# qwang-sj/qwen3-asr.cpp

Measured on AMD Instinct MI355X. Metric: RTFx (audio-sec/wall-sec) + decode tokens/sec, Qwen3-ASR-0.6B f16, higher is better.
Workload: dtype f16

## Files before the change

### qwen3-asr.cpp_amd/csrc/attention.hip

```cpp
#include <algorithm>
#include <type_traits>
#include <cstdlib>
#include <stdexcept>

#include "dev_common.h"
#include "fx_chain.h"
#include "fx_decode.h"
#include "kernels.h"

namespace qasr {

#define EKS 66
#define EVS 68

__global__ __launch_bounds__(256) void enc_attn_kernel(const float *__restrict__ qkv, const int *__restrict__ seg_start,
                                                       const int *__restrict__ seg_len, int D, uint16_t *__restrict__ out,
                                                       float *__restrict__ out32) {
    __shared__ __attribute__((aligned(16))) float Ks[64 * EKS];
    __shared__ __attribute__((aligned(16))) float Vs[64 * EVS];
    const int b = blockIdx.z, h = blockIdx.y;
    const int N = seg_len[b], r0 = seg_start[b];
    const int qblk = blockIdx.x * 64;
    if (qblk >= N) return;
    const int tid = threadIdx.x, lane = tid & 63, wid = tid >> 6;
// ... 512 lines not shown
#pragma unroll
                for (int i = 0; i < 4; i++) dst[d * 16 + 4 * g + i] = f_to_u16(o[d][i] * inv);
        }
    }
}

void launch_prefill_attention(const PrefillAttnArgs &a, hipStream_t s) {
    if (a.n_seq <= 0 || a.max_len <= 0) return;
    dim3 grid((a.max_len + 31) / 32, a.n_kv_head, a.n_seq);
    hipLaunchKernelGGL(prefill_attn_kernel, grid, dim3(256), 0, s, a);
}

#define DSPLIT 64
#define DWAVES 4

__device__ __forceinline__ void st_sc1_x4(float *p, float4 f) {
    const floatx4 v = {f.x, f.y, f.z, f.w};
    asm volatile("global_store_dwordx4 %0, %1, off sc1" ::"v"(p), "v"(v) : "memory");
}
__device__ __forceinline__ void ld_sc1_x4_burst5(const floatx4 *src, int tid, int n4, floatx4 *v) {
    const floatx4 *p[5];
#pragma unroll
    for (int j = 0; j < 5; j++) p[j] = src + min(tid + 256 * j, n4 - 1);
    asm volatile(
        "global_load_dwordx4 %0, %5, off sc1\n\t"
        "global_load_dwordx4 %1, %6, off sc1\n\t"
        "global_load_dwordx4 %2, %7, off sc1\n\t"
        "global_load_dwordx4 %3, %8, off sc1\n\t"
        "global_load_dwordx4 %4, %9, off sc1\n\t"
        "s_waitcnt vmcnt(0)"
        : "=&v"(v[0]), "=&v"(v[1]), "=&v"(v[2]), "=&v"(v[3]), "=&v"(v[4])
        : "v"(p[0]), "v"(p[1]), "v"(p[2]), "v"(p[3]), "v"(p[4])
        : "memory");
}
__device__ __forceinline__ void ld_sc1_x4_4(const uint16_t *p, u32x4 *v) {
    asm volatile(
        "global_load_dwordx4 %0, %4, off sc1\n\t"
        "global_load_dwordx4 %1, %4, off offset:1024 sc1\n\t"
        "global_load_dwordx4 %2, %4, off offset:2048 sc1\n\t"
        "global_load_dwordx4 %3, %4, off offset:3072 sc1\n\t"
        "s_waitcnt vmcnt(0)"
        : "=&v"(v[0]), "=&v"(v[1]), "=&v"(v[2]), "=&v"(v[3])
        : "v"(p)
        : "memory");
}

__device__ __forceinline__ half8 kv_load(const uint16_t *p, int nt) {
    return nt ? __builtin_nontemporal_load((const half8 *)p) : *(const half8 *)p;
}

template <int SPL>
struct alignas(16) SplitLds {
    uint16_t qs[2][128];
    uint16_t knew[128];
    uint16_t vnew[128];
    float sc[2][SPL];
    float ored[DWAVES * 4][2][128];
    float cml[2][2];
    int last;
};
template <int SPL, bool FUSED>
__device__ __forceinline__ void decode_attn_body(const DecodeAttnArgs a, const int sp, const int g, const int b, const int nsp,
                                                 SplitLds<SPL> &SL) {
    auto &qs = SL.qs;
    auto &knew = SL.knew;
    auto &vnew = SL.vnew;
    auto &sc = SL.sc;
    auto &ored = SL.ored;
    auto &cml = SL.cml;
    auto &last = SL.last;
    const int tid = threadIdx.x, lane = tid & 63, wid = tid >> 6;
    const int QD = a.n_head * 128, KD = a.n_kv_head * 128;
    const long blk = sp + (long)nsp * (g + (long)a.n_kv_head * b);
    auto mark = [&](int slot) {
        if (a.trace && tid == 0) a.trace[blk * 8 + slot] = rt_now();
    };
    mark(0);
    const float *raw = a.qkv + (long)b * (QD + 2 * KD);
    const float *src = wid < 2 ? raw + (2 * g + wid) * 128 : raw + QD + (wid - 2) * KD + g * 128;
    float x0 = 0.f, x1 = 0.f;
    if constexpr (!FUSED) { x0 = src[lane]; x1 = src[lane + 64]; }
    const float *nw = wid < 2 ? a.q_norm : a.k_norm;
    const float w0 = nw[lane], w1 = nw[lane + 64];
    if constexpr (FUSED)
        for (int i = 0; i < a.fuse_delay; i++) __builtin_amdgcn_s_sleep(8);
    const long cbase = ((long)b * a.n_kv_head + g) * a.max_ctx;
    uint16_t *kc = a.kc + cbase * 128, *vc = a.vc + cbase * 128;
    const int k0 = sp * SPL;
    const int sub = lane >> 4, dl = (lane & 15) * 8;
    const int q4 = lane >> 4, c16 = lane & 15;
    constexpr int KPW = SPL / DWAVES / 4;
    constexpr int TW = SPL / DWAVES / 16;
    const int kcap = FUSED ? a.max_ctx - 1 : min(a.pos[b], a.max_ctx - 1);
    half8 kk[TW][4], vv[KPW];
#pragma unroll
    for (int t = 0; t < TW; t++)
#pragma unroll
        for (int s4 = 0; s4 < 4; s4++) {
            const int key = min(k0 + wid * (SPL / DWAVES) + 16 * t + c16, kcap);
            kk[t][s4] = kv_load(kc + (long)key * 128 + 32 * s4 + 8 * q4, a.kv_nt);
        }
    if (FUSED && a.fx) {
        if (a.fx_vpf & 1) {
            const uint16_t *vt = a.vt + ((long)b * a.n_kv_head + g) * 128 * vt_ctx(a.max_ctx) + (long)(k0 / 8) * 1024;
#pragma unroll
            for (int i = 0; i < KPW; i++) vv[i] = *(const half8 *)(vt + (long)(i * 256 + tid) * 8);
        }
    } else if (!a.scores) {
#pragma unroll
        for (int i = 0; i < KPW; i++) {
            const int key = min(k0 + wid * (SPL / DWAVES) + i * 4 + sub, kcap);
            vv[i] = kv_load(vc + (long)key * 128 + dl, a.kv_nt);
        }
    }
    if (FUSED && a.gran) {
        const uint32_t tag = gran_tag(a.pos[b], a.layer);
        const unsigned long long *gp = a.gran + (src - raw) + lane;
        unsigned long long v0 = 0, v1 = 0;
        bool ok = false;
        for (int it = 0; it < a.poll_limit; it++) {
            v0 = __hip_atomic_load(gp, __ATOMIC_RELAXED, __HIP_MEMORY_SCOPE_AGENT);
            v1 = __hip_atomic_load(gp + 64, __ATOMIC_RELAXED, __HIP_MEMORY_SCOPE_AGENT);
            ok = (uint32_t)(v0 >> 32) == tag && (uint32_t)(v1 >> 32) == tag;
            if (__all(ok)) break;
            __builtin_amdgcn_s_sleep(2);
        }
        if (!__all(ok) && lane == 0) __hip_atomic_fetch_or(a.err, (unsigned)DEVERR_QKV_WAIT, __ATOMIC_RELAXED, __HIP_MEMORY_SCOPE_AGENT);
        x0 = __uint_as_float((uint32_t)v0);
        x1 = __uint_as_float((uint32_t)v1);
    } else if constexpr (FUSED) {
        if (tid == 0) {
            int ok = 0;
            for (int it = 0; it < a.poll_limit; it++) {
                if (__hip_atomic_load(a.qcnt + (g * 8 + (sp & 7)) * 16, __ATOMIC_RELAXED, __HIP_MEMORY_SCOPE_AGENT) >=
                    (a.qkv_need ? a.qkv_need : 64u)) {
                    ok = 1;
                    break;
                }
                __builtin_amdgcn_s_sleep(4);
            }
            if (a.fence) {
                __builtin_amdgcn_fence(__ATOMIC_ACQUIRE, "agent");
                asm volatile("s_waitcnt vmcnt(0)" ::: "memory");
            }
            if (!ok) __hip_atomic_fetch_or(a.err, (unsigned)DEVERR_QKV_WAIT, __ATOMIC_RELAXED, __HIP_MEMORY_SCOPE_AGENT);
        }
        __syncthreads();
        const uint32_t *sr = (const uint32_t *)src;
        x0 = __uint_as_float(__hip_atomic_load(sr + lane, __ATOMIC_RELAXED, __HIP_MEMORY_SCOPE_AGENT));
        x1 = __uint_as_float(__hip_atomic_load(sr + lane + 64, __ATOMIC_RELAXED, __HIP_MEMORY_SCOPE_AGENT));
    }
    const int pos = a.pos[b];
    const int nkv = pos + 1;
    const int k1 = min(nkv, k0 + SPL);
    const bool lastsp = sp == (nkv - 1) / SPL;
    const float2 cs = *(const float2 *)(a.rope + ((long)pos * 64 + lane) * 2);
    if (wid < 3) {
        const double ss = wave_sum_d((double)(x0 * x0) + (double)(x1 * x1));
        const float scale = 1.0f / sqrtf((float)(ss / 128.0) + a.eps);
        const float y0 = fmul_rn(fmul_rn(x0, scale), w0), y1 = fmul_rn(fmul_rn(x1, scale), w1);
        const uint16_t r0 = f_to_u16(y0 * cs.x - y1 * cs.y), r1 = f_to_u16(y0 * cs.y + y1 * cs.x);
        if (wid < 2) {
            qs[wid][lane] = r0;
            qs[wid][lane + 64] = r1;
        } else if (lastsp) {
            knew[lane] = r0; knew[lane + 64] = r1;
            kc[(long)pos * 128 + lane] = r0;
            kc[(long)pos * 128 + lane + 64] = r1;
        }
    } else if (lastsp) {
        const uint16_t v0 = f_to_u16(x0), v1 = f_to_u16(x1);
        vnew[lane] = v0; vnew[lane + 64] = v1;
        vc[(long)pos * 128 + lane] = v0;
        vc[(long)pos * 128 + lane + 64] = v1;
        uint16_t *t = a.vt + ((long)b * a.n_kv_head + g) * 128 * vt_ctx(a.max_ctx);
        t[vt_index(pos, lane)] = v0;
        t[vt_index(pos, lane + 64)] = v1;
    }
    __syncthreads();
    if (a.trace) { asm volatile("s_waitcnt vmcnt(0)" ::: "memory"); mark(1); }
    half8 qa[4];
#pragma unroll
    for (int s4 = 0; s4 < 4; s4++)
        qa[s4] = c16 < 2 ? *(const half8 *)&qs[c16][32 * s4 + 8 * q4] : half8{0, 0, 0, 0, 0, 0, 0, 0};
#pragma unroll
    for (int t = 0; t < TW; t++) {
        const int j = wid * (SPL / DWAVES) + 16 * t + c16;
        if (k0 + j == pos)
#pragma unroll
            for (int s4 = 0; s4 < 4; s4++) kk[t][s4] = *(const half8 *)&knew[32 * s4 + 8 * q4];
        floatx4 acc = {0.f, 0.f, 0.f, 0.f};
#pragma unroll
        for (int s4 = 0; s4 < 4; s4++) acc = __builtin_amdgcn_mfma_f32_16x16x32_f16(qa[s4], kk[t][s4], acc, 0, 0, 0);
        if (q4 == 0) {
            const bool ok = k0 + j < k1;
            sc[0][j] = ok ? acc[0] * a.scale : -INFINITY;
            sc[1][j] = ok ? acc[1] * a.scale : -INFINITY;
        }
    }
#pragma unroll
    for (int i = 0; i < KPW; i++) {
        const int j = wid * (SPL / DWAVES) + i * 4 + sub;
        if (k0 + j == pos) vv[i] = *(const half8 *)&vnew[dl];
    }
    __syncthreads();
    mark(6);
    if constexpr (FUSED) {
        if (a.fx) {
            const uint32_t tag = gran_tag(pos, a.layer);
            if (tid < 2 * SPL) {
                const int hh = tid / SPL, j = tid - hh * SPL;
                if (k0 + j < k1)
// ... 457 lines not shown
        fx_weights2(p ? fmaxf(Mp0, lh) : Mp0, p ? sv[2] : sv[0], p ? sv[3] : sv[1], x0, x1);
        const int k = k0 + 2 * p;
        if (k == kl) { C.fwl = x0; x0 = 0.0f; }
        if (k + 1 == kl) { C.fwl = x1; x1 = 0.0f; }
        *(float2 *)&C.fsc[(k >> 5) * FX_ST + (k & 31)] = make_float2(x0, x1);
        uint32_t m16 = kb << (4 * (lane & 3));
        m16 |= __shfl_xor(m16, 1, 64);
        m16 |= __shfl_xor(m16, 2, 64);
        const uint32_t bits = fx_chunk_bits(kb);
        if (p == 0) {
            if ((lane & 3) == 0) C.kmask[ch * (FX_PC / 16) + (lane >> 2)] = (uint16_t)m16;
            if ((lane & 7) == 7) C.gmax[ch * (FX_PC / DX_B) + (lane >> 3)] = Mi;
        }
        __builtin_amdgcn_fence(__ATOMIC_RELEASE, "workgroup");
        if (lane == 0) __hip_atomic_store(pb + 4 * ch + p, (unsigned char)(0x80u | bits), __ATOMIC_RELAXED, __HIP_MEMORY_SCOPE_WORKGROUP);
        if (tr && p == 0 && lane == 0 && (ch == 0 || ch == nch - 1)) {
            if (ch == 0) tr[2] = rt_now();
            if (ch == nch - 1) tr[3] = rt_now();
        }
    }
    if (p != 0) return;
    {
        uint32_t w = 0;
        for (int it = 0; it < a.poll_limit; it++) {
            w = __hip_atomic_load(pb + 4 * (nch - 1) + 1, __ATOMIC_RELAXED, __HIP_MEMORY_SCOPE_WORKGROUP);
            if (w & 0x80u) break;
            __builtin_amdgcn_s_sleep(1);
        }
        if (!(w & 0x80u) && lane == 0) __hip_atomic_fetch_or(a.err, (unsigned)DEVERR_SCORE_WAIT, __ATOMIC_RELAXED, __HIP_MEMORY_SCOPE_AGENT);
        __builtin_amdgcn_fence(__ATOMIC_ACQUIRE, "workgroup");
    }
    float term = 0.0f;
    if (lane * DX_B < nch * FX_PC) {
        const float *row = C.fsc + lane * FX_ST;
        const float wl = C.fwl;
        float Sl = 0.0f;
#pragma unroll
        for (int i = 0; i < DX_B; i += 4) {
            const floatx4 r = *(const floatx4 *)&row[i];
#pragma unroll
            for (int e = 0; e < 4; e++) Sl = __builtin_signbit(r[e]) ? fadd_rn(fmul_rn(Sl, -r[e]), 1.0f) : fadd_rn(fmul_rn(Sl, 1.0f), r[e]);
        }
        if (lane == (kl >> 5)) Sl = __builtin_signbit(wl) ? fadd_rn(fmul_rn(Sl, -wl), 1.0f) : fadd_rn(fmul_rn(Sl, 1.0f), wl);
        const float Ml = C.gmax[lane];
        term = Ml == -INFINITY ? 0.0f : Sl * expf(Ml - M);
    }
    const float S = wave_sum(term);
    if (lane == 0) C.S = S;
    __builtin_amdgcn_fence(__ATOMIC_RELEASE, "workgroup");
    if (lane == 0) __hip_atomic_store(&C.prog[DX_KC / FX_PC], FX_PUB, __ATOMIC_RELAXED, __HIP_MEMORY_SCOPE_WORKGROUP);
    if (tr && lane == 0) {
        tr[6] = rt_now();
        tr[7] = npoll;
    }
}
__device__ __forceinline__ uint32_t fx1_progress(const DecodeAttnArgs &a, ChainLds &C, const int i) {
    const uint32_t *pw = &C.prog[i];
    uint32_t w = (uint32_t)__builtin_amdgcn_readfirstlane((int)__hip_atomic_load(pw, __ATOMIC_RELAXED, __HIP_MEMORY_SCOPE_WORKGROUP));
    if (__builtin_expect((w & FX_PUB) != FX_PUB, 0)) {
        for (int it = 0; it < a.poll_limit; it++) {
            __builtin_amdgcn_s_sleep(1);
            w = (uint32_t)__builtin_amdgcn_readfirstlane((int)__hip_atomic_load(pw, __ATOMIC_RELAXED, __HIP_MEMORY_SCOPE_WORKGROUP));
            if ((w & FX_PUB) == FX_PUB) break;
        }
        if ((w & FX_PUB) != FX_PUB && (threadIdx.x & 63) == 0)
            __hip_atomic_fetch_or(a.err, (unsigned)DEVERR_SCORE_WAIT, __ATOMIC_RELAXED, __HIP_MEMORY_SCOPE_AGENT);
    }
    __builtin_amdgcn_fence(__ATOMIC_ACQUIRE, "workgroup");
    return w;
}
__device__ __forceinline__ void fx1_chain_body(const DecodeAttnArgs &a, const int c, ChainLds &C) {
    const int tid = threadIdx.x, lane = tid & 63, wid = __builtin_amdgcn_readfirstlane(tid >> 6);
    const int g = c % a.n_kv_head, hh = c / a.n_kv_head, head = 2 * g + hh;
    const int wu = wid & 1;
    const int d = 64 * wu + lane, loff = 8 * lane;
    const uint16_t *vt = a.vt + (long)g * 128 * vt_ctx(a.max_ctx) + 64 * wu * 8;
    unsigned long long *tr = a.trace ? a.trace + (4000L + c) * 8 : nullptr;
    auto mark = [&](int slot) {
        if (tr && tid == 0) tr[slot] = rt_now();
    };
    mark(0);
    const int pos = a.pos[0], n = pos + 1;
    if (tid <= DX_KC / FX_PC) C.prog[tid] = 0u;
    if (a.fx_vpf & 2) {
        typedef __attribute__((address_space(3))) void lds_void_c;
        typedef __attribute__((address_space(1))) void glb_void_c;
        lds_void_c *dst = (lds_void_c *)C.vpf[wid];
        for (int kb = wid >> 1; kb * 8 < n; kb += 2)
            __builtin_amdgcn_global_load_lds((glb_void_c *)(vt + (long)kb * 1024 + loff), dst, 16, 0, 0);
    }
    __syncthreads();
    if (wid >= 2) {
        fx1_gather_weights(a, head, n, C, wid - 2, tr);
    } else {
        const uint32_t tag = gran_tag(pos, a.layer);
        const int QD = a.n_head * 128, KD = a.n_kv_head * 128;
        const float *fsc = C.fsc;
        const uint16_t *kmask = C.kmask;
        const int nl = n - 1;
        if (a.trace && nl > 0) {
            (void)fx1_progress(a, C, 0);
            mark(1);
        }
        const unsigned long long ck0 = a.trace ? clock64() : 0ull;
        f16 acc = 0;
        {
            u32x4 va[DX_Q / 8], vb[DX_Q / 8];
            floatx4 wa, wb;
            const int lastb = nl > 0 ? (nl - 1) >> 3 : 0;
            const int nfull = nl > 0 ? (lastb + 1) >> 3 : 0;
            constexpr uint32_t QB = DX_Q / 8 * 2048;
            const __amdgpu_buffer_rsrc_t vrs = __builtin_amdgcn_make_buffer_rsrc((void *)vt, (short)0, lastb * 2048 + 1024, 0x00020000);
            const uint32_t voff = 16 * lane;
            int jt = 0;
            fx_loadQ(va, vt, loff, 0, lastb);
            uint32_t bm = 0;
            const float *wrow = fsc;
            const uint16_t *krow = kmask;
            for (; jt + 2 * DX_Q < nfull * DX_Q; jt += 2 * DX_Q, bm >>= 2, wrow += 2 * DX_Q / DX_B * FX_ST, krow += 2 * DX_Q / 16) {
                fx_loadQ_sb(vb, vrs, voff, (jt / DX_Q + 1) * QB);
                if ((jt & (FX_PC - 1)) == 0) {
                    bm = fx1_progress(a, C, jt / FX_PC);
                    fx_w8(wrow, 0, wa, wb);
                }
                fx_step1_lds_b(va, 0, wrow, krow, bm & 1u, acc, wa, wb);
                fx_loadQ_sb(va, vrs, voff, (jt / DX_Q + 2) * QB);
                fx_step1_lds_b(vb, DX_Q, wrow, krow, bm & 2u, acc, wa, wb);
            }
            for (int j0 = jt; j0 < nl; j0 += 2 * DX_Q, bm >>= 2) {
                fx_loadQ(vb, vt, loff, j0 + DX_Q, lastb);
                if ((j0 & (FX_PC - 1)) == 0) {
                    bm = fx1_progress(a, C, j0 / FX_PC);
                    fx_w8(fsc, j0, wa, wb);
                }
                fx_step1_lds_b(va, j0, fsc, kmask, bm & 1u, acc, wa, wb);
                if (j0 + DX_Q >= nl) break;
                fx_loadQ(va, vt, loff, j0 + 2 * DX_Q, lastb);
                fx_step1_lds_b(vb, j0 + DX_Q, fsc, kmask, bm & 2u, acc, wa, wb);
            }
        }
        const unsigned long long ck1 = a.trace ? clock64() : 0ull;
        uint16_t vnew = 0;
        {
            const unsigned long long *gp = a.gran + QD + KD + g * 128 + d;
            unsigned long long v = 0;
            bool ok = false;
            for (int it = 0; it < a.poll_limit; it++) {
                v = __hip_atomic_load(gp, __ATOMIC_RELAXED, __HIP_MEMORY_SCOPE_AGENT);
                ok = (uint32_t)(v >> 32) == tag;
                if (__all(ok)) break;
                __builtin_amdgcn_s_sleep(2);
            }
            if (!__all(ok) && lane == 0) __hip_atomic_fetch_or(a.err, (unsigned)DEVERR_QKV_WAIT, __ATOMIC_RELAXED, __HIP_MEMORY_SCOPE_AGENT);
            vnew = f_to_u16(__uint_as_float((uint32_t)v));
        }
        (void)fx1_progress(a, C, DX_KC / FX_PC);
        const float S = C.S;
        acc = fx_key_slow(acc, vnew, C.fwl);
        mark(4);
        if (a.trace && lane == 0) {
            a.trace[(4080L + c) * 8 + wid] = rt_now();
            a.trace[(4080L + c) * 8 + 2 + wid] = ck1 - ck0;
        }
        if (a.trace && tid == 0) {
            a.trace[(4040L + c) * 8 + 0] = ck0;
            a.trace[(4040L + c) * 8 + 1] = ck1;
            a.trace[(4040L + c) * 8 + 2] = (unsigned long long)n;
        }
        const float ov = (float)acc * (S == 0.0f ? 0.0f : 1.0f / S);
        const uint32_t h16 = f_to_u16(ov);
        const uint32_t hn = __shfl_xor(h16, 1, 64);
        uint16_t *out = a.out + head * 128 + d;
        if (a.att_done) {
            if ((lane & 1) == 0) __hip_atomic_store((uint32_t *)out, h16 | (hn << 16), __ATOMIC_RELAXED, __HIP_MEMORY_SCOPE_AGENT);
            asm volatile("s_waitcnt vmcnt(0)" ::: "memory");
        } else {
            *out = (uint16_t)h16;
        }
    }
    if (a.att_done) {
        __syncthreads();
        if (a.fence && tid == 0) {
            __builtin_amdgcn_fence(__ATOMIC_RELEASE, "agent");
            asm volatile("s_waitcnt vmcnt(0)" ::: "memory");
        }
        if (a.fence) __syncthreads();
        if (tid < 8) __hip_atomic_fetch_add(a.att_done + tid * 16, 1u, __ATOMIC_RELAXED, __HIP_MEMORY_SCOPE_AGENT);
    }
    mark(5);
    if (a.trace && tid == 0) {
        unsigned nk = 0, ng = 0;
        for (int i = 0; i < (n + FX_PC - 1) / FX_PC * (FX_PC / 16); i++) {
            const unsigned m = C.kmask[i];
            nk += __builtin_popcount(m);
            ng += ((m & 0xffu) != 0) + ((m >> 8) != 0);
        }
        a.trace[(4040L + c) * 8 + 3] = nk;
        a.trace[(4040L + c) * 8 + 4] = ng;
    }
}

template <int SPL>
__global__ __launch_bounds__(256) void qkv_attn1_kernel(GemvArgs q, DecodeAttnArgs a, GemvArgs o) {
    constexpr int K = 1024, NT = 2, RPW = 2;
    constexpr size_t RLB = sizeof(SplitLds<SPL>) > sizeof(ChainLds) ? sizeof(SplitLds<SPL>) : sizeof(ChainLds);
    __shared__ __attribute__((aligned(16))) unsigned char role_lds[RLB];
    stamp_start(a.stamp);
    if (blockIdx.x >= 512) {
        const int j = blockIdx.x - 512, nsp = a.grid_splits, nat = nsp * a.n_kv_head;
        const int nfx = fx_chain_wgs(a.fx, a.n_head);
        if (j >= nat + nfx) oproj1_body(o, a, j - nat - nfx);
        else if (j >= nat) fx1_chain_body(a, j - nat, *reinterpret_cast<ChainLds *>(role_lds));
        else decode_attn_body<SPL, true>(a, j / a.n_kv_head, j % a.n_kv_head, 0, nsp, *reinterpret_cast<SplitLds<SPL> *>(role_lds));
        stamp_end(a.stamp);
        return;
    }
    const int lane = threadIdx.x & 63, wid = threadIdx.x >> 6;
    const int grp = blockIdx.x >> 6, loc = blockIdx.x & 63;
    if (q.trace && threadIdx.x == 0) q.trace[blockIdx.x * 8] = rt_now();
    const int QD = a.n_head * 128, KD = a.n_kv_head * 128;
    const int rbase = loc < 32 ? grp * 256 + loc * 8 : loc < 48 ? QD + grp * 128 + (loc - 32) * 8 : QD + KD + grp * 128 + (loc - 48) * 8;
    const int row0 = rbase + wid * RPW;
    const uint32_t gtag = a.gran ? gran_tag(a.pos[0], a.layer) : 0u;
    half8 wv[RPW][NT];
#pragma unroll
    for (int r = 0; r < RPW; r++)
#pragma unroll
        for (int t = 0; t < NT; t++)
            wv[r][t] = __builtin_nontemporal_load((const half8 *)(q.W + (long)(row0 + r) * K + t * 512 + lane * 8));
    float xf[NT][8];
    if (q.embd_ids) {
        const uint16_t *er = q.embd + (long)q.embd_ids[0] * K;
#pragma unroll
        for (int t = 0; t < NT; t++) {
            const half8 h = *(const half8 *)(er + t * 512 + lane * 8);
#pragma unroll
            for (int e = 0; e < 8; e++) xf[t][e] = (float)h[e];
        }
        if (q.x_store && blockIdx.x == 0 && wid == 0)
#pragma unroll
            for (int t = 0; t < NT; t++)
#pragma unroll
                for (int e = 0; e < 8; e++)
                    __hip_atomic_store((uint32_t *)(q.x_store + t * 512 + lane * 8 + e), __float_as_uint(xf[t][e]), __ATOMIC_RELAXED,
                                       __HIP_MEMORY_SCOPE_AGENT);
    } else {
#pragma unroll
        for (int t = 0; t < NT; t++) {
            const float4 u = *(const float4 *)(q.x + t * 512 + lane * 8);
            const float4 v = *(const float4 *)(q.x + t * 512 + lane * 8 + 4);
            xf[t][0] = u.x; xf[t][1] = u.y; xf[t][2] = u.z; xf[t][3] = u.w;
            xf[t][4] = v.x; xf[t][5] = v.y; xf[t][6] = v.z; xf[t][7] = v.w;
        }
    }
    double ss = 0.0;
#pragma unroll
    for (int t = 0; t < NT; t++)
#pragma unroll
        for (int e = 0; e < 8; e++) ss += (double)(xf[t][e] * xf[t][e]);
    ss = wave_sum_d(ss);
    const float scale = 1.0f / sqrtf((float)(ss / K) + q.eps);
#pragma unroll
    for (int t = 0; t < NT; t++) {
        const float4 u = *(const float4 *)(q.norm_w + t * 512 + lane * 8);
        const float4 v = *(const float4 *)(q.norm_w + t * 512 + lane * 8 + 4);
        const float w[8] = {u.x, u.y, u.z, u.w, v.x, v.y, v.z, v.w};
#pragma unroll
        for (int e = 0; e < 8; e++) xf[t][e] = (float)f2h(fmul_rn(fmul_rn(xf[t][e], scale), w[e]));
    }
#pragma unroll
    for (int r = 0; r < RPW; r++) {
        float acc = 0.f;
#pragma unroll
        for (int t = 0; t < NT; t++)
#pragma unroll
            for (int e = 0; e < 8; e++) acc = fmaf((float)wv[r][t][e], xf[t][e], acc);
        acc = wave_sum(acc);
        if (a.gran) {
            if (lane == 0)
                __hip_atomic_store(a.gran + row0 + r, ((unsigned long long)gtag << 32) | __float_as_uint(acc), __ATOMIC_RELAXED,
                                   __HIP_MEMORY_SCOPE_AGENT);
        } else if (lane == 0) {
            __hip_atomic_store((uint32_t *)(q.out_f32 + row0 + r), __float_as_uint(acc), __ATOMIC_RELAXED, __HIP_MEMORY_SCOPE_AGENT);
        }
    }
    if (a.gran) {
        if (q.trace && threadIdx.x == 0) q.trace[blockIdx.x * 8 + 1] = rt_now();
        stamp_end(a.stamp);
        return;
    }
    asm volatile("s_waitcnt vmcnt(0)" ::: "memory");
    __syncthreads();
    if (a.fence && threadIdx.x == 0) {
        __builtin_amdgcn_fence(__ATOMIC_RELEASE, "agent");
        asm volatile("s_waitcnt vmcnt(0)" ::: "memory");
    }
    if (a.fence) __syncthreads();
    if (threadIdx.x < 8)
        __hip_atomic_fetch_add(a.qcnt + (grp * 8 + threadIdx.x) * 16, 1u, __ATOMIC_RELAXED, __HIP_MEMORY_SCOPE_AGENT);
    if (q.trace && threadIdx.x == 0) q.trace[blockIdx.x * 8 + 1] = rt_now();
    stamp_end(a.stamp);
}

static int split1(int spl1, int grid_splits) { return spl1 == 64 || spl1 == 128 ? spl1 : grid_splits >= 30 ? 128 : 64; }

int launch_qkv_attention1(const GemvArgs &q, const DecodeAttnArgs &a, const GemvArgs *o, const FuseCfg &cfg, hipStream_t s, bool dry) {
    if (!cfg.qkv || !cfg.err || a.B != 1 || !a.qcnt || q.M != 1 || q.K != 1024 || q.Wd || !q.norm_w || q.xh || q.bias || q.res ||
        a.out32 || a.outq || q.N != a.n_head * 128 + 2 * a.n_kv_head * 128 || a.n_head != 2 * a.n_kv_head || a.n_kv_head * 64 != 512)
        return 0;
    const int spl1 = split1(cfg.spl1, a.grid_splits);
    const int ns = (a.grid_splits * DSPLIT + spl1 - 1) / spl1;
    const bool with_o = cfg.o && o && a.att_done && o->M == 1 && o->K == 2048 && o->N == 1024 && o->xh && o->res &&
                        !o->Wd && !o->bias && !o->norm_w && o->xh == a.out;
    if (a.fx && (!a.gran || !a.sgran || ns * spl1 > DX_KC)) return 0;
    const int nfx = fx_chain_wgs(a.fx, a.n_head);
    const int slots = spl1 == 128 ? cfg.slots_qkv128 : cfg.slots_qkv64;
    const int o_blocks = 1024 / OPROJ_ROWS;
    const bool fit_o = 512 + ns * a.n_kv_head + nfx + o_blocks <= slots;
    if (512 + ns * a.n_kv_head + nfx > slots) return 0;
    const bool with_o2 = with_o && fit_o;
    if (dry) return with_o2 ? 2 : 1;
    const dim3 grid(512 + ns * a.n_kv_head + nfx + (with_o2 ? o_blocks : 0));
    DecodeAttnArgs ad = a;
    ad.fuse_delay = cfg.qkv_delay;
    ad.oproj_delay = cfg.o_delay;
    ad.poll_limit = cfg.poll_limit;
    ad.fence = cfg.fence;
    ad.err = cfg.err;
    ad.grid_splits = ns;
    ad.fx_vpf = cfg.fx_vpf;
    if (!with_o2) ad.att_done = nullptr;
    const GemvArgs qa = q;
    const GemvArgs oa = with_o2 ? *o : GemvArgs{};
    if (spl1 == 128) hipLaunchKernelGGL(qkv_attn1_kernel<128>, grid, dim3(256), 0, s, qa, ad, oa);
    else hipLaunchKernelGGL(qkv_attn1_kernel<DSPLIT>, grid, dim3(256), 0, s, qa, ad, oa);
    return with_o2 ? 2 : 1;
}

void launch_decode_attention(const DecodeAttnArgs &a, hipStream_t s) {
    if (a.B <= 0) return;
    if (a.B <= 8) {
        if (split1(a.spl1, a.grid_splits) == 128) {
            const int g2 = (a.grid_splits * DSPLIT + 127) / 128;
            hipLaunchKernelGGL(decode_attn_kernel<128>, dim3(g2, a.n_kv_head, a.B), dim3(256), 0, s, a);
        } else {
            hipLaunchKernelGGL(decode_attn_kernel<DSPLIT>, dim3(a.grid_splits, a.n_kv_head, a.B), dim3(256), 0, s, a);
        }
    } else if (a.stream_blocks > 0 && a.n_head == 2 * a.n_kv_head && a.n_kv_head * a.B >= a.stream_blocks / 2) {
        hipLaunchKernelGGL(decode_attn_seq_kernel<0>, dim3(a.n_kv_head, a.B), dim3(256), 0, s, a);
    } else {
        if (a.spl_batch == 128) {
            const int g2 = (a.grid_splits * DSPLIT + 127) / 128;
            hipLaunchKernelGGL(decode_attn_kernel<128>, dim3(g2, a.n_kv_head, a.B), dim3(256), 0, s, a);
        } else {
            const int g4 = (a.grid_splits * DSPLIT + 255) / 256;
            hipLaunchKernelGGL(decode_attn_kernel<256>, dim3(g4, a.n_kv_head, a.B), dim3(256), 0, s, a);
        }
    }
}

bool launch_decode_attention_exact_seq(const DecodeAttnArgs &a, hipStream_t s) {
    const size_t lds = (size_t)2 * a.max_ctx * sizeof(float);
    if (!a.fx_seq || a.B <= 8 || a.stream_blocks <= 0 || a.n_head != 2 * a.n_kv_head || a.n_kv_head * a.B < a.stream_blocks / 2 ||
        lds > 32768)
        return false;
    hipLaunchKernelGGL(decode_attn_seq_kernel<1>, dim3(a.n_kv_head, a.B), dim3(256), lds, s, a);
    return true;
}

int fused_slots_ffn();

void fused_slots(FuseCfg &cfg) {
    auto slots_of = [](const void *kernel) {
        int nb = 0, dev = 0, cus = 0;
        if (hipGetDevice(&dev) != hipSuccess || hipDeviceGetAttribute(&cus, hipDeviceAttributeMultiprocessorCount, dev) != hipSuccess ||
            hipOccupancyMaxActiveBlocksPerMultiprocessor(&nb, kernel, 256, 0) != hipSuccess)
            return 0;
        return nb * cus;
    };
    cfg.slots_qkv64 = slots_of(reinterpret_cast<const void *>(qkv_attn1_kernel<DSPLIT>));
    cfg.slots_qkv128 = slots_of(reinterpret_cast<const void *>(qkv_attn1_kernel<128>));
    cfg.slots_ffn = fused_slots_ffn();
    cfg.slots_stream = decode_stream_slots();
}

int decode_split_len() { return DSPLIT; }
int decode_max_splits() { return 256; }

}
```

### qwen3-asr.cpp_amd/csrc/engine.hip

```cpp
#include <memory>

#include "engine_impl.h"

using namespace qasr;
using namespace qasr::eng;

static thread_local std::string g_err;

int qasr::eng::fail(int code, const std::string &msg) {
    g_err = msg;
    return code;
}

int qasr::eng::declined_check(const char *stage) {
    std::string msg;
    if (qasr::take_declined(&msg)) return fail(QASR_ERR_STATE, std::string(stage) + ": " + msg);
    return 0;
}

struct FuseOption {
    const char *name, *env;
    int FuseCfg::*field;
};
static const std::vector<FuseOption> &fuse_options() {
    static const std::vector<FuseOption> v = {
        {"fuse_ffn", "QASR_FUSE_FFN", &FuseCfg::ffn},          {"fuse_qkv", "QASR_FUSE_QKV", &FuseCfg::qkv},
        {"fuse_o", "QASR_FUSE_O", &FuseCfg::o},
        {"ffn_delay", "QASR_FFN_DELAY", &FuseCfg::ffn_delay},
        {"ffn_wdelay", "QASR_FFN_WDELAY", &FuseCfg::ffn_wdelay}, {"qkv_delay", "QASR_FUSE_DELAY", &FuseCfg::qkv_delay},
        {"o_delay", "QASR_FUSE_ODELAY", &FuseCfg::o_delay},    {"att_spl1", "QASR_ATT_SPL1", &FuseCfg::spl1},
        {"poll_limit", "QASR_POLL_LIMIT", &FuseCfg::poll_limit}, {"handoff_fence", "QASR_HANDOFF_FENCE", &FuseCfg::fence},
        {"fa_exact_prefill", "QASR_FA_EXACT_PREFILL", &FuseCfg::fa_exact_prefill},
        {"enc_attn_f32", "QASR_ENC_ATTN_F32", &FuseCfg::enc_attn_f32},
        {"gemm_regs", "QASR_GEMM_REGS", &FuseCfg::gemm_regs},
        {"gran", "QASR_GRAN", &FuseCfg::gran},
        {"fa_exact_decode", "QASR_FA_EXACT_DECODE", &FuseCfg::fa_exact_decode},
        {"fx_vpf", "QASR_FX_VPF", &FuseCfg::fx_vpf},
        {"att_stream", "QASR_ATT_STREAM", &FuseCfg::att_stream},
        {"skinny", "QASR_SKINNY", &FuseCfg::skinny},
        {"att_spl", "QASR_ATT_SPL", &FuseCfg::att_spl},
        {"kv_nt", "QASR_KV_NT", &FuseCfg::kv_nt},
        {"lmh", "QASR_LMH", &FuseCfg::lmh},
        {"fx_seq", "QASR_FX_SEQ", &FuseCfg::fx_seq},
        {"skinny_inf", "QASR_SKINNY_INF", &FuseCfg::skinny_inf},
        {"skinny_wdef", "QASR_SKINNY_WDEF", &FuseCfg::skinny_wdef},
        {"refill_group", "QASR_REFILL_GROUP", &FuseCfg::refill_group},
        {"live_prefix", "QASR_LIVE_PREFIX", &FuseCfg::live_prefix},
        {"staged_wrap", "QASR_STAGED_WRAP", &FuseCfg::staged_wrap},
        {"poison_scratch", "QASR_POISON_SCRATCH", &FuseCfg::poison},
        {"token_logprobs", "QASR_TOKEN_LOGPROBS", &FuseCfg::token_logprobs},
        {"top_k", "QASR_TOP_K", &FuseCfg::top_k},
        {"lmh_topk", "QASR_LMH_TOPK", &FuseCfg::lmh_topk},
        {"beam_width", "QASR_BEAM_WIDTH", &FuseCfg::beam_width},
        {"sample_slices", "QASR_SAMPLE_SLICES", &FuseCfg::sample_slices},
    };
    return v;
}

int qasr::eng::reset_counters(qasr_ctx *c) {
    HIPCHK(hipMemsetAsync(c->d_ffncnt, 0, c->ffncnt_bytes(), c->st));
    HIPCHK(hipMemsetAsync(c->d_qcnt, 0, c->qcnt_bytes(), c->st));
    HIPCHK(hipMemsetAsync(c->d_attdone, 0, c->attdone_bytes(), c->st));
    HIPCHK(hipMemsetAsync(c->d_counter, 0, c->counter_bytes(), c->st));
    HIPCHK(hipMemsetAsync(c->d_done, 0, qasr_ctx::kDoneBytes, c->st));
    HIPCHK(hipMemsetAsync(c->d_amax, 0, c->amax_bytes(), c->st));
    return 0;
}

int qasr::eng::reset_granules(qasr_ctx *c) {
    HIPCHK(hipMemsetAsync(c->d_gran, 0, c->gran_bytes(), c->st));
    HIPCHK(hipMemsetAsync(c->d_sgran, 0, c->sgran_bytes(), c->st));
    return 0;
}

int qasr::eng::check_dev_err(qasr_ctx *c) {
    unsigned e = 0;
    HIPCHK(hipMemcpyAsync(&e, c->d_err, 4, hipMemcpyDeviceToHost, c->st));
    HIPCHK(hipStreamSynchronize(c->st));
    if (!e) return 0;
    HIPCHK(hipMemsetAsync(c->d_err, 0, 4, c->st));
    const int rc = reset_counters(c);
    if (rc) return rc;
    HIPCHK(hipStreamSynchronize(c->st));
    std::string what;
    if (e & DEVERR_QKV_WAIT) what += " attention<-QKV";
    if (e & DEVERR_O_WAIT) what += " o-proj<-attention";
    if (e & DEVERR_FFN_WAIT) what += " down<-gate/up";
    if (e & DEVERR_SCORE_WAIT) what += " chain<-scores";
    return fail(QASR_ERR_DEVICE, "fused decode launch: an in-launch wait timed out (" + what.substr(1) +
                                     "); outputs of this call are invalid (another process or context sharing the GPU?)");
}

std::mutex &qasr::eng::device_lock(int device) {
    static std::mutex m[64];
    return m[(unsigned)device % 64];
}

int qasr::eng::dev_alloc(qasr_ctx *c, void **p, size_t bytes) {
    HIPCHK(hipMalloc(p, bytes ? bytes : 256));
    c->owned.push_back({*p, bytes});
    return 0;
}

int qasr::eng::ensure(qasr_ctx *c, DevBuf &b, size_t bytes) {
    if (b.n >= bytes && b.p) return 0;
    if (b.p) {
        HIPCHK(hipStreamSynchronize(c->st));
        for (auto it = c->owned.begin(); it != c->owned.end(); ++it)
            if (it->p == b.p) { c->owned.erase(it); break; }
        HIPCHK(hipFree(b.p));
        b.p = nullptr;
    }
    size_t n = std::max<size_t>(bytes + bytes / 4, 4096);
    HIPCHK(hipMalloc(&b.p, n));
    b.n = n;
    c->owned.push_back({b.p, n});
    if (c->fuse.poison) HIPCHK(hipMemsetAsync(b.p, 0xFF, n, c->st));
    return 0;
}

// ... 329 lines not shown
```

### qwen3-asr.cpp_amd/csrc/kernels.h

```cpp
#pragma once

#include <string>

#include <hip/hip_runtime.h>
#include <stdint.h>

namespace qasr {

struct MelClip {
    long pcm_off;
    int n;
    int TF;
    long tmp_off;
    long out_off;
};
void launch_mel(const float *pcm, const MelClip *clips, int n_clips, const int2 *blocks, int n_blocks,
                const double2 *tw, const double *hann, const float *filt, double *tmp, unsigned long long *cmax,
                float *out, hipStream_t s);
int mel_frames_per_block();

struct ResampleClip {
    long in_off;
    long out_off;
    int n_in, n_out;
// ... 38 lines not shown
    const uint16_t *A; int lda;
    const uint16_t *W; int ldw;
    int M, N, K;
    const ChunkDesc *chunks; const int *row_start; int n_chunks; int C;
    const float *bias;
    const float *res; int ldr;
    float *out_f32; int ldo;
    uint16_t *out_f16; int ldo16;
    const uint16_t *gelu;
    const float *pe; const int *pe_pos;
    unsigned long long *amax;
    int n_valid;
    const int8_t *Aq; const float *Ad; int ldad;
    const int8_t *Wq; const uint16_t *Wd;
    int regs_staged;
    int no_skinny;
    int skinny_inflight;
    int8_t *out_q; float *out_d; int ldoq;
    int wdef;
};
void launch_gemm(int amode, int epi, const GemmArgs &g, hipStream_t s);
void note_declined(const char *what, int mode, int epi);
void note_declined_shape(const char *what, int M, int N, int K);
bool take_declined(std::string *msg);
void note_kernel(const char *family, int n, int a = 0, int b = 0, int c = 0, int d = 0, int e = 0);
bool take_kernel(std::string *tag);
bool launch_gemm_skinny(int epi, const GemmArgs &g, hipStream_t s);
bool launch_gemm_skinny_q8(int epi, const GemmArgs &g, hipStream_t s);
void launch_gemm_q8(int epi, const GemmArgs &g, hipStream_t s);
void launch_quantize_q8(const float *x32, const uint16_t *x16, int ldx, int M, int K, int gather_C, int8_t *q, float *d,
                        hipStream_t s);

struct ScoreHeadArgs {
    const uint16_t *A; int lda;
    const uint16_t *W; int ldw;
    int R, N, K, n_valid;
    const int32_t *target;
    float *lp;
    int32_t *gid;
    float *glp;
    void *scratch;
    int cols_fast;
};
size_t score_head_scratch(int R, int N);
bool launch_score_head(const ScoreHeadArgs &a, hipStream_t s);

struct GemvArgs {
    const float *x; int ldx;
    const uint16_t *xh; int ldxh;
    const float *norm_w; float eps;
    const uint16_t *W; int K, N, M;
    const uint16_t *Wd;
    const float *bias;
    const float *res; int ldr;
    float *out_f32; int ldo;
    uint16_t *out_f16; int ldo16;
    unsigned long long *amax;
    const int32_t *embd_ids; const uint16_t *embd; float *x_store;
    unsigned int *done; int32_t *tok_out; int32_t *hist; int hist_stride; int *step; int *pos;
    unsigned long long *trace;
    unsigned int *zero8;
    unsigned long long *stamp;
    int *nkv;
    int n_valid;
    int keep_step;
    unsigned long long *lp_part; float *lp_out; float *lp_hist;
    unsigned long long *tk_part; int32_t *tk_out; float *tk_lp; int32_t *tk_hist; float *tk_lphist; int tk_k;
};
void launch_gemv(int epi, const GemvArgs &g, hipStream_t s);
bool launch_lmhead_batch(const GemvArgs &g, hipStream_t s);
int lmhead_grid();
bool launch_gemv1(int epi, const GemvArgs &g, hipStream_t s);

enum DevErr : unsigned {
    DEVERR_QKV_WAIT = 1u,
    DEVERR_O_WAIT = 2u,
    DEVERR_FFN_WAIT = 4u,
    DEVERR_SCORE_WAIT = 8u,
};
struct FuseCfg {
    int ffn = 1, qkv = 1, o = 1;
    int ffn_delay = 4, ffn_wdelay = 16;
    int qkv_delay = 10, o_delay = 32;
    int spl1 = 0;
    int poll_limit = 1 << 20;
    int fence = 0;
    int enc_attn_f32 = 0;
    int gemm_regs = 0;
    int gran = 1;
    int fa_exact_prefill = 1;
    int fa_exact_decode = 1;
    int fx_vpf = 2;
    int slots_ffn = 0, slots_qkv64 = 0, slots_qkv128 = 0;
    int att_stream = 1;
    int skinny = 1;
    int att_spl = 256;
    int kv_nt = 1;
    int slots_stream = 0;
    int fx_seq = 1;
    int lmh = 1;
    int skinny_inf = 1;
    int skinny_wdef = 1;
    int refill_group = 0;
    int live_prefix = 0;
    int staged_wrap = 0;
    int poison = 0;
    int sample_slices = 0;
    int token_logprobs = 0;
    int lmh_topk = 1;
    int top_k = 0;
    int beam_width = 0;
    unsigned int *err = nullptr;
};
void fused_slots(FuseCfg &cfg);
struct FfnCtl {
    unsigned int *cnt, *cnt_next;
    unsigned int *err;
    int wdelay, delay, poll_limit, fence;
};
bool launch_ffn1(const GemvArgs &gu, const GemvArgs &dn, unsigned int *cnt, unsigned int *cnt_next, const FuseCfg &cfg,
                 hipStream_t s, bool dry = false);

void launch_layernorm_f16(const float *x, int M, int D, const float *w, const float *b, float eps, uint16_t *y, hipStream_t s,
                          float *y32 = nullptr);
void launch_rmsnorm_f16(const float *x, int ldx, const int *row_idx, int M, int D, const float *w, float eps,
                        uint16_t *y, hipStream_t s, float *y32 = nullptr);
void launch_rmsnorm_q8(const float *x, int ldx, int M, int D, const float *w, float eps, int8_t *yq, float *yd, hipStream_t s);

void launch_enc_attention(const float *qkv, const int *seg_start, const int *seg_len, int n_seg, int max_len,
                          int D, int H, uint16_t *out, hipStream_t s, float *out32 = nullptr, bool f32_mfma = false);

constexpr long kKvPadRows = 256;
__host__ __device__ inline int vt_ctx(int max_ctx) { return (max_ctx + 63) / 64 * 64 + 384; }
__host__ __device__ inline long vt_index(int k, int d) { return ((long)(k >> 3) * 128 + d) * 8 + (k & 7); }

struct QkvPostArgs {
    const float *qkv; int rows;
    const int *row_seq; const int *row_pos;
    const float *q_norm, *k_norm; float eps;
    const float *rope;
    int n_head, n_kv_head;
    uint16_t *q_out;
    uint16_t *kc, *vc;
    int max_ctx;
    uint16_t *vt;
    float *q32, *k32;
};
void launch_qkv_post(const QkvPostArgs &a, hipStream_t s);

struct PrefillAttnArgs {
    const uint16_t *q;
    const uint16_t *kc, *vc;
    const int *seq_row0; const int *seq_len; const int *seq_slot; int n_seq; int max_len;
    int n_head, n_kv_head, max_ctx;
    float scale;
    uint16_t *out;
    float *out32;
    int8_t *outq; float *outd;
    const float *q32, *k32;
    const int *seq_pos0;
};
void launch_prefill_attention(const PrefillAttnArgs &a, hipStream_t s);
void launch_prefill_attention_exact(const PrefillAttnArgs &a, hipStream_t s);
hipError_t check_expf_nonpos(unsigned long long *mismatches);

__host__ __device__ inline int sgran_ld(int max_ctx) { return (max_ctx + 63) / 64 * 64; }
__host__ __device__ inline uint32_t gran_tag(int pos, int layer) { return ((uint32_t)(pos + 1) << 5) | (uint32_t)layer; }

struct DecodeAttnArgs {
    const float *qkv;
    const float *q_norm, *k_norm; float eps;
    const float *rope;
    const int *pos;
    uint16_t *kc, *vc;
    uint16_t *vt;
    const int *seq_slot;
    int B, n_head, n_kv_head, max_ctx, max_splits;
    int grid_splits;
    float scale;
    float *part;
    unsigned int *counter;
    uint16_t *out;
    float *out32;
    int8_t *outq; float *outd;
    unsigned long long *trace;
    unsigned int *qcnt;
    int fuse_delay;
    unsigned int *att_done;
    int oproj_delay;
    int poll_limit;
    int fence;
    unsigned int *err;
    int spl1;
    unsigned long long *stamp;
    unsigned int qkv_need;
    float *scores;
    unsigned long long *gran;
    int layer;
    int stream_blocks;
    int spl_batch;
    int kv_nt;
    int fx_seq;
    int fx;
    unsigned long long *sgran;
    int fx_vpf;
};
void launch_decode_attention_exact(const DecodeAttnArgs &a, hipStream_t s);
bool launch_decode_attention_exact_seq(const DecodeAttnArgs &a, hipStream_t s);

void launch_decode_attention(const DecodeAttnArgs &a, hipStream_t s);
int launch_qkv_attention1(const GemvArgs &q, const DecodeAttnArgs &a, const GemvArgs *o, const FuseCfg &cfg, hipStream_t s,
                          bool dry = false);
int decode_split_len();
int decode_max_splits();

void launch_embed(const int32_t *ids, int rows, const uint16_t *embd, int hidden, const float *audio,
                  const int *row_audio , float *x, hipStream_t s);
void launch_argmax_finish(const unsigned long long *amax, int B, int32_t *ids, int32_t *hist, int hist_stride,
                          const int *step, hipStream_t s);
void launch_fill_u64(unsigned long long *p, int n, unsigned long long v, hipStream_t s);
void launch_token_logprob(const float *logits, int ld, int B, int n_valid, const int32_t *tok, const int *step, float *lp_out,
                          float *lp_hist, int hist_stride, hipStream_t s, int src_div = 1);
constexpr int TOPK_MAX = 8;
bool launch_topk_rows(const float *logits, int ld, int B, int n_valid, int K, const int *step, int32_t *tk_ids, float *tk_lp,
                      int32_t *tk_hist_ids, float *tk_hist_lp, int hist_stride, hipStream_t s);
void launch_gather_rows(const float *src, const int *idx, int rows, int D, float *dst, hipStream_t s);
void launch_step_advance(int *row_pos, int *n_kv, int *step, int B, hipStream_t s);

struct KvForkArgs {
    uint16_t *kc, *vc, *vt;
    int layers, n_kv_head, max_ctx, slots;
    const int *parent, *from, *to;
    int B, group, blocks;
};
bool launch_kv_fork(const KvForkArgs &a, hipStream_t s);
struct BeamSelectArgs {
    const int32_t *tk_id; const float *tk_lp;
    float *cum;
    int *fin_row, *fin_t; float *fin_sum, *fin_lp;
    int *n_fin, *done, *t;
    const int *P;
    int32_t *tok;
    int *parent, *from, *to;
    int *h_par; int32_t *h_id; float *h_lp;
    int hist_stride, hist_base;
    int W, G;
    const int32_t *eos;
};
bool launch_beam_select(const BeamSelectArgs &a, hipStream_t s);

struct SampleScalars {
    float inv_T, cut;
    uint32_t seed_lo, seed_hi;
};
struct SampleArgs {
    const float *logits; int ld, n_valid;
    const int32_t *greedy;
    const int *clip, *sample;
    int *t;
    const SampleScalars *sc;
    unsigned long long *skey;
    int32_t *tok;
    int32_t *hist; int hist_stride; const int *step;
    float *key_out;
    int R, src_div;
};
int sample_slices(int R, int n_valid);
bool launch_sample(const SampleArgs &a, int slices, hipStream_t s);
void launch_sample_gumbel_dump(uint32_t n0, uint32_t n, float *out, hipStream_t s);

constexpr int kConstrainNgramMax = 8, kConstrainBiasMax = 1024, kConstrainVocabMax = 1 << 20;
struct ConstrainParams {
    int ngram;
    float p, inv_p;
    int last_n;
    int n_bias;
};
constexpr int kPhraseWalkMax = 15;
struct PhraseTrie {
    int n_nodes;
    const int32_t *child_off;
    const int32_t *tok, *dst;
    const float *bonus;
};
struct ConstrainArgs {
    float *logits; int ld, n_valid;
    const int32_t *greedy;
    const int32_t *hist_in; int hist_stride; const int *step;
// ... 16 lines not shown
```

Measured before the change: 296.6.

## Stagger fused QKV/attention memory traffic and skip redundant K-row polling

```diff
diff --git a/qwen3-asr.cpp_amd/csrc/attention.hip b/qwen3-asr.cpp_amd/csrc/attention.hip
--- a/qwen3-asr.cpp_amd/csrc/attention.hip
+++ b/qwen3-asr.cpp_amd/csrc/attention.hip
@@ -618,8 +618,10 @@
     if constexpr (!FUSED) { x0 = src[lane]; x1 = src[lane + 64]; }
     const float *nw = wid < 2 ? a.q_norm : a.k_norm;
     const float w0 = nw[lane], w1 = nw[lane + 64];
-    if constexpr (FUSED)
-        for (int i = 0; i < a.fuse_delay; i++) __builtin_amdgcn_s_sleep(8);
+    if constexpr (FUSED) {
+        const int nd = a.fuse_delay + (sp * SPL / 256) * a.k_stagger;
+        for (int i = 0; i < nd; i++) __builtin_amdgcn_s_sleep(8);
+    }
     const long cbase = ((long)b * a.n_kv_head + g) * a.max_ctx;
     uint16_t *kc = a.kc + cbase * 128, *vc = a.vc + cbase * 128;
     const int k0 = sp * SPL;
@@ -650,20 +652,23 @@
         }
     }
     if (FUSED && a.gran) {
-        const uint32_t tag = gran_tag(a.pos[b], a.layer);
-        const unsigned long long *gp = a.gran + (src - raw) + lane;
-        unsigned long long v0 = 0, v1 = 0;
-        bool ok = false;
-        for (int it = 0; it < a.poll_limit; it++) {
-            v0 = __hip_atomic_load(gp, __ATOMIC_RELAXED, __HIP_MEMORY_SCOPE_AGENT);
-            v1 = __hip_atomic_load(gp + 64, __ATOMIC_RELAXED, __HIP_MEMORY_SCOPE_AGENT);
-            ok = (uint32_t)(v0 >> 32) == tag && (uint32_t)(v1 >> 32) == tag;
-            if (__all(ok)) break;
-            __builtin_amdgcn_s_sleep(2);
-        }
-        if (!__all(ok) && lane == 0) __hip_atomic_fetch_or(a.err, (unsigned)DEVERR_QKV_WAIT, __ATOMIC_RELAXED, __HIP_MEMORY_SCOPE_AGENT);
-        x0 = __uint_as_float((uint32_t)v0);
-        x1 = __uint_as_float((uint32_t)v1);
+        const int gpos = a.pos[b];
+        const uint32_t tag = gran_tag(gpos, a.layer);
+        if (wid < 2 || sp == gpos / SPL) {
+            const unsigned long long *gp = a.gran + (src - raw) + lane;
+            unsigned long long v0 = 0, v1 = 0;
+            bool ok = false;
+            for (int it = 0; it < a.poll_limit; it++) {
+                v0 = __hip_atomic_load(gp, __ATOMIC_RELAXED, __HIP_MEMORY_SCOPE_AGENT);
+                v1 = __hip_atomic_load(gp + 64, __ATOMIC_RELAXED, __HIP_MEMORY_SCOPE_AGENT);
+                ok = (uint32_t)(v0 >> 32) == tag && (uint32_t)(v1 >> 32) == tag;
+                if (__all(ok)) break;
+                __builtin_amdgcn_s_sleep(2);
+            }
+            if (!__all(ok) && lane == 0) __hip_atomic_fetch_or(a.err, (unsigned)DEVERR_QKV_WAIT, __ATOMIC_RELAXED, __HIP_MEMORY_SCOPE_AGENT);
+            x0 = __uint_as_float((uint32_t)v0);
+            x1 = __uint_as_float((uint32_t)v1);
+        }
     } else if constexpr (FUSED) {
         if (tid == 0) {
             int ok = 0;
@@ -1287,17 +1292,24 @@
     mark(0);
     const int pos = a.pos[0], n = pos + 1;
     if (tid <= DX_KC / FX_PC) C.prog[tid] = 0u;
-    if (a.fx_vpf & 2) {
-        typedef __attribute__((address_space(3))) void lds_void_c;
-        typedef __attribute__((address_space(1))) void glb_void_c;
-        lds_void_c *dst = (lds_void_c *)C.vpf[wid];
-        for (int kb = wid >> 1; kb * 8 < n; kb += 2)
-            __builtin_amdgcn_global_load_lds((glb_void_c *)(vt + (long)kb * 1024 + loff), dst, 16, 0, 0);
-    }
+    typedef __attribute__((address_space(3))) void lds_void_c;
+    typedef __attribute__((address_space(1))) void glb_void_c;
+    lds_void_c *vdst = (lds_void_c *)C.vpf[wid];
+    const int npf = a.vt_stagger > 0 ? min(n, FX_PC) : n;
+    const int vhalf = (a.fx_vpf & 4) ? 1 : 0;
+    if (a.fx_vpf & 2)
+        for (int kb = (wid >> 1) + 2 * hh * vhalf; kb * 8 < npf; kb += 2 + 2 * vhalf)
+            __builtin_amdgcn_global_load_lds((glb_void_c *)(vt + (long)kb * 1024 + loff), vdst, 16, 0, 0);
     __syncthreads();
     if (wid >= 2) {
         fx1_gather_weights(a, head, n, C, wid - 2, tr);
     } else {
+        if ((a.fx_vpf & 2) && npf < n) {
+            for (int i = 0; i < a.vt_stagger; i++) __builtin_amdgcn_s_sleep(8);
+            for (int kb = FX_PC / 8; kb * 8 < n; kb++)
+                __builtin_amdgcn_global_load_lds((glb_void_c *)(vt + (long)kb * 1024 + loff), vdst, 16, 0, 0);
+            __builtin_amdgcn_s_waitcnt(0x0F70);
+        }
         const uint32_t tag = gran_tag(pos, a.layer);
         const int QD = a.n_head * 128, KD = a.n_kv_head * 128;
         const float *fsc = C.fsc;
@@ -1421,12 +1433,12 @@
         return;
     }
     const int lane = threadIdx.x & 63, wid = threadIdx.x >> 6;
-    const int grp = blockIdx.x >> 6, loc = blockIdx.x & 63;
     if (q.trace && threadIdx.x == 0) q.trace[blockIdx.x * 8] = rt_now();
-    const int QD = a.n_head * 128, KD = a.n_kv_head * 128;
-    const int rbase = loc < 32 ? grp * 256 + loc * 8 : loc < 48 ? QD + grp * 128 + (loc - 32) * 8 : QD + KD + grp * 128 + (loc - 48) * 8;
-    const int row0 = rbase + wid * RPW;
-    const uint32_t gtag = a.gran ? gran_tag(a.pos[0], a.layer) : 0u;
+    const int qb = blockIdx.x;
+    const int grp = qb < 256 ? qb >> 5 : (qb & 127) >> 4;
+    const int row0 = qb * 8 + wid * RPW;
+    if (qb >= 256)
+        for (int i = 0; i < a.kvw_delay; i++) __builtin_amdgcn_s_sleep(8);
     half8 wv[RPW][NT];
 #pragma unroll
     for (int r = 0; r < RPW; r++)
@@ -1473,6 +1485,7 @@
 #pragma unroll
         for (int e = 0; e < 8; e++) xf[t][e] = (float)f2h(fmul_rn(fmul_rn(xf[t][e], scale), w[e]));
     }
+    const uint32_t gtag = gran_tag(a.pos[0], a.layer);
 #pragma unroll
     for (int r = 0; r < RPW; r++) {
         float acc = 0.f;
@@ -1534,6 +1547,9 @@
     ad.err = cfg.err;
     ad.grid_splits = ns;
     ad.fx_vpf = cfg.fx_vpf;
+    ad.kvw_delay = max(cfg.kvw_delay, 0);
+    ad.k_stagger = max(cfg.k_stagger, 0);
+    ad.vt_stagger = max(cfg.vt_stagger, 0);
     if (!with_o2) ad.att_done = nullptr;
     const GemvArgs qa = q;
     const GemvArgs oa = with_o2 ? *o : GemvArgs{};
diff --git a/qwen3-asr.cpp_amd/csrc/engine.hip b/qwen3-asr.cpp_amd/csrc/engine.hip
--- a/qwen3-asr.cpp_amd/csrc/engine.hip
+++ b/qwen3-asr.cpp_amd/csrc/engine.hip
@@ -36,6 +36,9 @@
         {"gran", "QASR_GRAN", &FuseCfg::gran},
         {"fa_exact_decode", "QASR_FA_EXACT_DECODE", &FuseCfg::fa_exact_decode},
         {"fx_vpf", "QASR_FX_VPF", &FuseCfg::fx_vpf},
+        {"kvw_delay", "QASR_KVW_DELAY", &FuseCfg::kvw_delay},
+        {"k_stagger", "QASR_K_STAGGER", &FuseCfg::k_stagger},
+        {"vt_stagger", "QASR_VT_STAGGER", &FuseCfg::vt_stagger},
         {"att_stream", "QASR_ATT_STREAM", &FuseCfg::att_stream},
         {"skinny", "QASR_SKINNY", &FuseCfg::skinny},
         {"att_spl", "QASR_ATT_SPL", &FuseCfg::att_spl},
diff --git a/qwen3-asr.cpp_amd/csrc/kernels.h b/qwen3-asr.cpp_amd/csrc/kernels.h
--- a/qwen3-asr.cpp_amd/csrc/kernels.h
+++ b/qwen3-asr.cpp_amd/csrc/kernels.h
@@ -144,6 +144,9 @@
     int ffn = 1, qkv = 1, o = 1;
     int ffn_delay = 4, ffn_wdelay = 16;
     int qkv_delay = 10, o_delay = 32;
+    int kvw_delay = 3;
+    int k_stagger = 6;
+    int vt_stagger = 0;
     int spl1 = 0;
     int poll_limit = 1 << 20;
     int fence = 0;
@@ -152,7 +155,7 @@
     int gran = 1;
     int fa_exact_prefill = 1;
     int fa_exact_decode = 1;
-    int fx_vpf = 2;
+    int fx_vpf = 6;
     int slots_ffn = 0, slots_qkv64 = 0, slots_qkv128 = 0;
     int att_stream = 1;
     int skinny = 1;
@@ -266,6 +269,7 @@
     int fx;
     unsigned long long *sgran;
     int fx_vpf;
+    int kvw_delay, k_stagger, vt_stagger;
 };
 void launch_decode_attention_exact(const DecodeAttnArgs &a, hipStream_t s);
 bool launch_decode_attention_exact_seq(const DecodeAttnArgs &a, hipStream_t s);
```

Result: faster. 305.5 (median of 6 runs) (+3.0%).
